# hzeller/timg

Hardware: NVIDIA H100
Metric: Mpixels/s scale+dither+sixel-encode @4K→cell (higher is better)
Workload: dtype u8/f32

## Files before the change

timg_b200/csrc/sixel.cu:

```cuda
#include <cstdlib>

#include "sixel.cuh"

namespace b200timg {

constexpr int PT = 1024;

__device__ __forceinline__ int pick_plane(int d0, int d1, int d2) {
    const double lum[3] = {0.2989, 0.5866, 0.1145};
    const int spreads[3] = {d0 << 3, d1 << 3, d2 << 3};
    int plane = 0; double best = 0.0;
#pragma unroll
    for (int p = 0; p < 3; ++p) { const double sp = lum[p] * (double)spreads[p]; if (sp > best) { plane = p; best = sp; } }
    return plane;
}

template <bool SMEM_TABLES>
__global__ void __launch_bounds__(PT)
sixel_palette_kernel(const uint32_t *__restrict__ fb, int w, int h, SixelWork W) {
    extern __shared__ uint32_t s_hist[];
    __shared__ uint32_t s_w[PT / 32];
    __shared__ int b_ind[256], b_col[256], b_med[256], t_ind[256], t_col[256], t_med[256];
    __shared__ uint32_t b_sum[256], b_low[256], t_sum[256], t_low[256];
    __shared__ int s_mn[3], s_mx[3];
// ... 349 lines not shown
constexpr int DW_MAX = 24;
constexpr int DCH = 16;
constexpr int DIN_STRIDE = DCH + 1;
constexpr int DOUT_STRIDE = 20;
constexpr int DWARP_SMEM = 2 * 32 * DIN_STRIDE * 4 + 32 * DOUT_STRIDE;

__global__ void __launch_bounds__(DW_MAX * 32)
sixel_dither_kernel(const uint32_t *__restrict__ fb, int w, int h, int nwarps, SixelWork W) {
    extern __shared__ __align__(16) uint8_t s_dyn[];
    __shared__ uint32_t s_pal[256];
    __shared__ volatile int s_progress[2048];
    const int f = blockIdx.x;
    const SixelFrameHdr *hdr = W.hdr + f;
    if (!hdr->diffuse) return;
    const int tid = threadIdx.x, lane = tid & 31, wid = tid >> 5;
    const int nthreads = nwarps * 32;
    uint8_t *s_lut = s_dyn;
    for (int i = tid; i < 32768 / 4; i += nthreads)
        reinterpret_cast<uint32_t *>(s_lut)[i] = reinterpret_cast<const uint32_t *>(W.lut + (long long)f * 32768)[i];
    for (int i = tid; i < 256; i += nthreads) s_pal[i] = hdr->palette[i];
    for (int i = tid; i < W.nb32; i += nthreads) s_progress[i] = 0;
    __syncthreads();
    uint32_t *s_in = reinterpret_cast<uint32_t *>(s_dyn + 32768 + (size_t)wid * DWARP_SMEM);
    uint8_t *s_out = reinterpret_cast<uint8_t *>(s_in + 2 * 32 * DIN_STRIDE);
    const uint32_t *frame = fb + (long long)f * w * h;
    uint8_t *index = W.index + (long long)f * w * h;
    uint32_t *bnd = W.boundary + (long long)f * W.nb32 * w;
    const int hrow = lane >> 4, hcol = lane & 15;

    for (int band = wid; band < W.nb32; band += nwarps) {
        const int y = band * 32 + lane;
        const bool row_ok = y < h;
        const bool last_row = (y == h - 1);
        const uint32_t *bin = band > 0 ? bnd + (long long)(band - 1) * w : nullptr;
        uint32_t *bout = bnd + (long long)band * w;
        uint32_t last_e = EZ;
        FsErr up_m1, up_0, up_p1, own, e_first;
        up_m1.zero(); up_0.zero(); up_p1.zero(); own.zero(); e_first.zero();
        const int steps = w + 62, nchunks = (steps + DCH - 1) / DCH;
        uint32_t pre[16];
        auto load_chunk = [&](int c) {
#pragma unroll
            for (int i = 0; i < 16; ++i) {
                const int r = 2 * i + hrow, yy = band * 32 + r, x = c * DCH - 2 * r + hcol;
                pre[i] = (yy < h && x >= 0 && x < w) ? frame[(long long)yy * w + x] : 0u;
            }
        };
        auto store_chunk = [&](int c) {
            uint32_t *t = s_in + (c & 1) * 32 * DIN_STRIDE;
#pragma unroll
            for (int i = 0; i < 16; ++i) t[(2 * i + hrow) * DIN_STRIDE + hcol] = pre[i];
        };
        load_chunk(0); store_chunk(0);
        __syncwarp();
        for (int c = 0; c < nchunks; ++c) {
            const int t0 = c * DCH;
            if (c + 1 < nchunks) load_chunk(c + 1);
            uint32_t binreg = EZ;
            if (band > 0) {
                const int need = min(w, t0 + DCH + 1);
                if (lane == 0) { while (s_progress[band - 1] < need) __nanosleep(32); __threadfence_block(); }
                __syncwarp();
                const int bx = t0 + 1 + lane;
                if (lane < DCH && bx < w) binreg = __ldcg(bin + bx);
                if (c == 0 && lane == 0) up_p1.unpack(__ldcg(bin));
            }
            const uint32_t *tin = s_in + (c & 1) * 32 * DIN_STRIDE + lane * DIN_STRIDE;
            uint32_t bkeep = EZ;
            const bool interior = (t0 - 62 >= 1) && (t0 + DCH - 1 <= w - 2) && (band * 32 + 31 < h - 1);
            if (interior) {
#pragma unroll 4
                for (int j = 0; j < DCH; ++j) {
                    uint32_t recv = __shfl_up_sync(0xffffffffu, last_e, 1);
                    const uint32_t b0 = __shfl_sync(0xffffffffu, binreg, j);
                    if (lane == 0) recv = b0;
                    up_m1 = up_0; up_0 = up_p1; up_p1.unpack(recv);
                    const uint32_t px = tin[j];
                    int v[3] = {(int)(px & 0xff), (int)((px >> 8) & 0xff), (int)((px >> 16) & 0xff)};
#pragma unroll
                    for (int ch = 0; ch < 3; ++ch) {
                        v[ch] = fs_add(v[ch], up_m1, ch, 1);
                        v[ch] = fs_add(v[ch], up_0, ch, 5);
                        v[ch] = fs_add(v[ch], up_p1, ch, 3);
                        v[ch] = fs_add(v[ch], own, ch, 7);
                    }
                    const uint32_t cell = ((uint32_t)(v[0] >> 3) << 10) | ((uint32_t)(v[1] >> 3) << 5) | (uint32_t)(v[2] >> 3);
                    const uint32_t ci = s_lut[cell];
                    const uint32_t pal = s_pal[ci];
                    own.set(v[0] - (int)(pal & 0xff), v[1] - (int)((pal >> 8) & 0xff), v[2] - (int)((pal >> 16) & 0xff));
                    last_e = own.pack();
                    s_out[lane * DOUT_STRIDE + j] = (uint8_t)ci;
                    const uint32_t e31 = __shfl_sync(0xffffffffu, last_e, 31);
                    if (lane == j) bkeep = e31;
                }
            } else {
#pragma unroll 2
                for (int j = 0; j < DCH; ++j) {
                    const int t = t0 + j, x = t - 2 * lane;
                    uint32_t recv = __shfl_up_sync(0xffffffffu, last_e, 1);
                    const uint32_t b0 = __shfl_sync(0xffffffffu, binreg, j);
                    if (lane == 0) recv = b0;
                    up_m1 = up_0; up_0 = up_p1; up_p1.unpack(recv);
                    uint32_t ci = 0;
                    if (x >= 0 && x < w && row_ok) {
                        const uint32_t px = tin[j];
                        int v[3] = {(int)(px & 0xff), (int)((px >> 8) & 0xff), (int)((px >> 16) & 0xff)};
#pragma unroll
                        for (int ch = 0; ch < 3; ++ch) {
                            v[ch] = fs_add(v[ch], up_m1, ch, 1);
                            v[ch] = fs_add(v[ch], up_0, ch, 5);
                            v[ch] = fs_add(v[ch], up_p1, ch, 3);
                            if (x == w - 1) v[ch] = fs_add(v[ch], e_first, ch, 3);
                            v[ch] = fs_add(v[ch], own, ch, 7);
                        }
                        const uint32_t cell = ((uint32_t)(v[0] >> 3) << 10) | ((uint32_t)(v[1] >> 3) << 5) | (uint32_t)(v[2] >> 3);
                        ci = s_lut[cell];
                        const uint32_t pal = s_pal[ci];
                        if (x < w - 1 && !last_row) own.set(v[0] - (int)(pal & 0xff), v[1] - (int)((pal >> 8) & 0xff), v[2] - (int)((pal >> 16) & 0xff));
                        else own.zero();
                        if (x == 0) e_first = own;
                        last_e = own.pack();
                    } else if (x >= w) {
                        last_e = EZ;
                    }
                    s_out[lane * DOUT_STRIDE + j] = (uint8_t)ci;
                    const uint32_t e31 = __shfl_sync(0xffffffffu, last_e, 31);
                    if (lane == j) bkeep = e31;
                }
            }
            __syncwarp();
#pragma unroll
            for (int i = 0; i < 16; ++i) {
                const int r = 2 * i + hrow, yy = band * 32 + r, x = t0 - 2 * r + hcol;
                if (yy < h && x >= 0 && x < w) index[(long long)yy * w + x] = s_out[r * DOUT_STRIDE + hcol];
            }
            {
                const int x = t0 + lane - 62;
                if (lane < DCH && x >= 0 && x < w) __stcg(bout + x, bkeep);
                __threadfence_block();
                __syncwarp();
                const int done = min(w, t0 + DCH - 62);
                if (lane == 0 && done > 0) s_progress[band] = done;
            }
            if (c + 1 < nchunks) store_chunk(c + 1);
            __syncwarp();
        }
    }
}

__device__ __forceinline__ uint32_t ndig4(uint32_t v) { return 1u + (v >= 10u) + (v >= 100u) + (v >= 1000u); }
__device__ __forceinline__ char *put_num4(char *o, uint32_t v) {
    const uint32_t d3 = v / 1000u, r3 = v - d3 * 1000u, d2 = r3 / 100u, r2 = r3 - d2 * 100u, d1 = r2 / 10u, d0 = r2 - d1 * 10u;
    if (v >= 1000u) *o++ = (char)('0' + d3);
    if (v >= 100u) *o++ = (char)('0' + d2);
    if (v >= 10u) *o++ = (char)('0' + d1);
    *o++ = (char)('0' + d0);
    return o;
}
__device__ __forceinline__ uint32_t rle_len(uint32_t n) { return n > 3u ? 2u + ndig4(n) : n; }
__device__ __forceinline__ char *put_rle(char *o, uint32_t n, char ch) {
    if (n > 3u) { *o++ = '!'; o = put_num4(o, n); *o++ = ch; }
    else { if (n > 0u) *o++ = ch; if (n > 1u) *o++ = ch; if (n > 2u) *o++ = ch; }
    return o;
}

constexpr int ET = 512, EW = ET / 32;
__device__ __forceinline__ uint32_t ent_pack(uint32_t c, uint32_t x, uint32_t bits) { return (c << 18) | (x << 6) | bits; }

struct EmitGeom { int w, h, cols_per_warp; };

template <typename F>
__device__ __forceinline__ void walk_runs(const uint32_t *sorted, int lo, int hi, int n, F emit) {
    int i = lo;
    uint32_t prev = 0; bool have_prev = false;
    if (i > 0 && i < hi) { prev = sorted[i - 1]; have_prev = true; }
    while (i < hi) {
        const uint32_t e = sorted[i];
        if (have_prev && e == prev + 64u) { prev = e; ++i; continue; }
        uint32_t cur = e, L = 1;
        while (i + (int)L < n && sorted[i + L] == cur + 64u) { cur += 64u; ++L; }
        const uint32_t c = e >> 18, x = (e >> 6) & 4095u;
        const bool same_colour = have_prev && (prev >> 18) == c;
        emit(c, e & 63u, same_colour ? x - ((prev >> 6) & 4095u) - 1u : x, L, !same_colour);
        prev = cur; have_prev = true;
        i += (int)L;
    }
}

__global__ void __launch_bounds__(ET)
sixel_emit_kernel(EmitGeom G, SixelWork W) {
    extern __shared__ uint32_t s_sorted[];
    __shared__ uint32_t s_cnt[EW][256];
    __shared__ uint32_t s_mask[EW * 256];
    __shared__ uint32_t s_w[ET / 32];
    const int band = blockIdx.x, f = blockIdx.y, tid = threadIdx.x, lane = tid & 31, wid = tid >> 5;
    const int w = G.w;
    const SixelFrameHdr *hdr = W.hdr + f;
    const uint8_t *idx = W.index + ((long long)f * G.h + (long long)band * 6) * w;

    for (int i = tid; i < EW * 256; i += ET) { (&s_cnt[0][0])[i] = 0; s_mask[i] = 0; }
    __syncthreads();

    const int x_lo = wid * G.cols_per_warp, x_hi = min(w, x_lo + G.cols_per_warp);
    uint32_t *cnt = s_cnt[wid];
    for (int x = x_lo + lane; x < x_hi; x += 32) {
        uint32_t col[6], bits[6];
        const uint32_t valid = column_entries(idx, w, x, col, bits);
#pragma unroll
        for (int s = 0; s < 6; ++s) if (valid & (1u << s)) atomicAdd(&cnt[col[s]], 1u);
    }
    __syncthreads();
    uint32_t tot_c = 0;
    if (tid < 256) for (int k = 0; k < EW; ++k) tot_c += s_cnt[k][tid];
    uint32_t n_ent; const uint32_t cb = block_excl_scan<ET>(tid < 256 ? tot_c : 0, s_w, n_ent);
    if (tid < 256) {
        uint32_t run = cb;
        for (int k = 0; k < EW; ++k) { const uint32_t v = s_cnt[k][tid]; s_cnt[k][tid] = run; run += v; }
    }
    __syncthreads();
    uint32_t *M = s_mask + wid * 256;
    const uint32_t lt = (1u << lane) - 1;
    for (int x0 = x_lo; x0 < x_hi; x0 += 32) {
        const int x = x0 + lane;
        uint32_t col[6], bits[6];
        const uint32_t valid = x < x_hi ? column_entries(idx, w, x, col, bits) : 0u;
#pragma unroll
        for (int s = 0; s < 6; ++s) if (valid & (1u << s)) atomicOr(&M[col[s]], 1u << lane);
        __syncwarp();
        uint32_t mk[6];
#pragma unroll
        for (int s = 0; s < 6; ++s)
            if (valid & (1u << s)) {
                mk[s] = M[col[s]];
                s_sorted[cnt[col[s]] + __popc(mk[s] & lt)] = ent_pack(col[s], (uint32_t)x, bits[s]);
            }
        __syncwarp();
#pragma unroll
        for (int s = 0; s < 6; ++s)
            if ((valid & (1u << s)) && (mk[s] & lt) == 0) { cnt[col[s]] += (uint32_t)__popc(mk[s]); M[col[s]] = 0; }
        __syncwarp();
    }
    __syncthreads();
    const int n = (int)n_ent;
    const uint32_t minc = s_sorted[0] >> 18;
    const int per = (n + ET - 1) / ET, lo = min(n, tid * per), hi = min(n, lo + per);
    uint32_t local = 0;
    walk_runs(s_sorted, lo, hi, n, [&](uint32_t c, uint32_t, uint32_t gap, uint32_t len, bool first) {
        local += rle_len(gap) + rle_len(len) + (first ? 1u + ndig4(c) + (c != minc ? 1u : 0u) : 0u);
    });
    uint32_t band_total; uint32_t at = block_excl_scan<ET>(local, s_w, band_total);
    if (tid == 0) W.band_bytes[(long long)f * W.nbands + band] = band_total;
    char *o = W.scratch + ((size_t)f * W.nbands + band) * W.band_cap + at;
    walk_runs(s_sorted, lo, hi, n, [&](uint32_t c, uint32_t bits, uint32_t gap, uint32_t len, bool first) {
        if (first) { if (c != minc) *o++ = '$'; *o++ = '#'; o = put_num4(o, c); }
        o = put_rle(o, gap, '?');
        o = put_rle(o, len, (char)('?' + bits));
    });
}

constexpr int SLOT_WORDS = 22;
constexpr int STASH_STEPS = 6;
constexpr uint32_t SLOT_MAX = 4 * (SLOT_WORDS - 3);
static_assert(SLOT_WORDS * ET >= 2 * EW * 256, "the slots alias the sort's tables");

struct DecTable { uint32_t v[4096]; };
constexpr DecTable make_dec_table() {
    DecTable t{};
    for (uint32_t n = 0; n < 4096; ++n) {
        uint32_t s = 0, m = n, nd = 0;
        do { s = (s << 8) | (0x30u + m % 10u); m /= 10u; ++nd; } while (m);
        t.v[n] = s;
    }
    return t;
}
__device__ const DecTable k_dec = make_dec_table();
__device__ __forceinline__ uint32_t dec4(uint32_t v, uint32_t &nd) {
    const uint32_t s = __ldg(&k_dec.v[v]);
    nd = 4u - ((uint32_t)__clz((int)s) >> 3);
    return s;
}
__device__ __forceinline__ unsigned long long rle_piece4(uint32_t n, uint32_t ch, uint32_t &len) {
    if (n > 3u) {
        uint32_t nd;
        const uint32_t d = dec4(n, nd);
        len = 2u + nd;
        return 0x21ull | ((unsigned long long)d << 8) | ((unsigned long long)ch << (8u * (1u + nd)));
    }
    len = n;
    return (unsigned long long)((ch * 0x010101u) & ((1u << (8u * n)) - 1u));
}
__device__ __forceinline__ void slot_append(uint32_t *slot, uint32_t &pos, uint32_t &cur, unsigned long long v, uint32_t len) {
    const uint32_t sh = 8u * (pos & 3u);
    const uint32_t lo = (uint32_t)v, hi = (uint32_t)(v >> 32);
    const uint32_t w0 = cur | (lo << sh);
    const uint32_t w1 = __funnelshift_l(lo, hi, sh);
    const uint32_t w2 = sh ? (hi >> (32u - sh)) : 0u;
    uint32_t *p = slot + min(pos >> 2, (uint32_t)(SLOT_WORDS - 3)) * ET;
    p[0] = w0; p[ET] = w1; p[2 * ET] = w2;
    const uint32_t np = pos + len, adv = (np >> 2) - (pos >> 2);
    cur = adv == 0u ? w0 : (adv == 1u ? w1 : w2);
    pos = np;
}

__global__ void __launch_bounds__(ET, 2)
sixel_emit1b_kernel(EmitGeom G, SixelWork W) {
    extern __shared__ uint32_t s_sorted[];
    __shared__ uint32_t s_tab[SLOT_WORDS * ET];
    __shared__ uint32_t s_w[ET / 32];
    const int band = blockIdx.x, f = blockIdx.y, tid = threadIdx.x, lane = tid & 31, wid = tid >> 5;
    const int w = G.w;
    const uint8_t *idx = W.index + ((long long)f * G.h + (long long)band * 6) * w;

    for (int i = tid; i < 2 * EW * 256; i += ET) s_tab[i] = 0;
    __syncthreads();
    const int x_lo = wid * G.cols_per_warp, x_hi = min(w, x_lo + G.cols_per_warp);
    uint32_t *cnt = s_tab + wid * 256, *M = s_tab + EW * 256 + wid * 256;
    const bool stash = G.cols_per_warp <= 32 * STASH_STEPS;
    uint32_t k0[STASH_STEPS], k1[STASH_STEPS], k2[STASH_STEPS];
    if (stash) {
#pragma unroll
        for (int t = 0; t < STASH_STEPS; ++t) {
            const int x = x_lo + 32 * t + lane;
            k0[t] = k1[t] = k2[t] = 0;
            if (x < x_hi) {
                uint32_t col[6], bits[6];
                const uint32_t valid = column_entries(idx, w, x, col, bits);
#pragma unroll
                for (int s = 0; s < 6; ++s) if (valid & (1u << s)) atomicAdd(&cnt[col[s]], 1u);
                k0[t] = col[0] | (col[1] << 8) | (col[2] << 16) | (col[3] << 24);
                k1[t] = col[4] | (col[5] << 8) | (valid << 16) | (bits[5] << 22);
                k2[t] = bits[0] | (bits[1] << 6) | (bits[2] << 12) | (bits[3] << 18) | (bits[4] << 24);
            }
        }
    } else {
        for (int x = x_lo + lane; x < x_hi; x += 32) {
            uint32_t col[6], bits[6];
            const uint32_t valid = column_entries(idx, w, x, col, bits);
#pragma unroll
            for (int s = 0; s < 6; ++s) if (valid & (1u << s)) atomicAdd(&cnt[col[s]], 1u);
        }
    }
    __syncthreads();
    uint32_t tot_c = 0;
    if (tid < 256) for (int k = 0; k < EW; ++k) tot_c += s_tab[k * 256 + tid];
    uint32_t n_ent; const uint32_t cb = block_excl_scan<ET>(tid < 256 ? tot_c : 0, s_w, n_ent);
    if (tid < 256) {
        uint32_t run = cb;
        for (int k = 0; k < EW; ++k) { const uint32_t v = s_tab[k * 256 + tid]; s_tab[k * 256 + tid] = run; run += v; }
    }
    __syncthreads();
    const uint32_t lt = (1u << lane) - 1;
    auto scatter_step = [&](int x, uint32_t valid, const uint32_t *col, const uint32_t *bits) {
#pragma unroll
        for (int s = 0; s < 6; ++s) if (valid & (1u << s)) atomicOr(&M[col[s]], 1u << lane);
        __syncwarp();
        uint32_t mk[6];
#pragma unroll
        for (int s = 0; s < 6; ++s)
            if (valid & (1u << s)) {
                mk[s] = M[col[s]];
                s_sorted[cnt[col[s]] + __popc(mk[s] & lt)] = ent_pack(col[s], (uint32_t)x, bits[s]);
            }
        __syncwarp();
#pragma unroll
        for (int s = 0; s < 6; ++s)
            if ((valid & (1u << s)) && (mk[s] & lt) == 0) { cnt[col[s]] += (uint32_t)__popc(mk[s]); M[col[s]] = 0; }
        __syncwarp();
    };
    if (stash) {
#pragma unroll
        for (int t = 0; t < STASH_STEPS; ++t) {
            if (x_lo + 32 * t < x_hi) {
                const uint32_t col[6] = {k0[t] & 255u, (k0[t] >> 8) & 255u, (k0[t] >> 16) & 255u, k0[t] >> 24, k1[t] & 255u, (k1[t] >> 8) & 255u};
                const uint32_t bits[6] = {k2[t] & 63u, (k2[t] >> 6) & 63u, (k2[t] >> 12) & 63u, (k2[t] >> 18) & 63u, (k2[t] >> 24) & 63u, (k1[t] >> 22) & 63u};
                scatter_step(x_lo + 32 * t + lane, (k1[t] >> 16) & 63u, col, bits);
            }
        }
    } else {
        for (int x0 = x_lo; x0 < x_hi; x0 += 32) {
            const int x = x0 + lane;
            uint32_t col[6], bits[6];
            const uint32_t valid = x < x_hi ? column_entries(idx, w, x, col, bits) : 0u;
            scatter_step(x, valid, col, bits);
        }
    }
    __syncthreads();
    const int n = (int)n_ent;
    const uint32_t minc = s_sorted[0] >> 18;
    const int per = (n + ET - 1) / ET, lo = min(n, tid * per), hi = min(n, lo + per);
    uint32_t *slot = s_tab + tid;
    uint32_t pos = 0, cur = 0;
    bool ovf = false;
    walk_runs(s_sorted, lo, hi, n, [&](uint32_t c, uint32_t bits, uint32_t gap, uint32_t len, bool first) {
        uint32_t pl;
        if (first) {
            uint32_t nd;
            unsigned long long v = 0x23ull | ((unsigned long long)dec4(c, nd) << 8);
            pl = 1u + nd;
            if (c != minc) { v = 0x24ull | (v << 8); ++pl; }
            ovf |= pos > SLOT_MAX;
            slot_append(slot, pos, cur, v, pl);
        }
        uint32_t rl;
        const unsigned long long gv = rle_piece4(gap, 0x3fu, pl), rv = rle_piece4(len, 0x3fu + bits, rl);
        ovf |= pos > SLOT_MAX;
        if (pl + rl <= 8u) {
            slot_append(slot, pos, cur, gv | (rv << (8u * pl)), pl + rl);
        } else {
            slot_append(slot, pos, cur, gv, pl);
            ovf |= pos > SLOT_MAX;
            slot_append(slot, pos, cur, rv, rl);
        }
    });
    const uint32_t local = pos;
    uint32_t band_total; const uint32_t at = block_excl_scan<ET>(local, s_w, band_total);
    if (tid == 0) W.band_bytes[(long long)f * W.nbands + band] = band_total;
    char *o = W.scratch + ((size_t)f * W.nbands + band) * W.band_cap + at;
    if (!ovf) {
        const uint32_t head = min(local, (4u - (at & 3u)) & 3u);
        const uint32_t w0 = slot[0];
        for (uint32_t k = 0; k < head; ++k) o[k] = (char)(w0 >> (8u * k));
        const uint32_t nw = (local - head) >> 2;
        uint32_t *dw = reinterpret_cast<uint32_t *>(o + head);
        uint32_t a = w0;
        for (uint32_t j = 0; j < nw; ++j) {
            const uint32_t b = slot[(j + 1) * ET];
            dw[j] = __funnelshift_r(a, b, 8u * head);
            a = b;
        }
        const uint32_t done = head + 4u * nw;
        for (uint32_t k = done; k < local; ++k) o[k] = (char)(slot[(k >> 2) * ET] >> (8u * (k & 3u)));
    } else {
        walk_runs(s_sorted, lo, hi, n, [&](uint32_t c, uint32_t bits, uint32_t gap, uint32_t len, bool first) {
            if (first) { if (c != minc) *o++ = '$'; *o++ = '#'; o = put_num4(o, c); }
            o = put_rle(o, gap, '?');
            o = put_rle(o, len, (char)('?' + bits));
        });
    }
}

__global__ void __launch_bounds__(256)
sixel_layout_kernel(int w, int h, SixelWork W) {
    __shared__ uint32_t s_w[8];
    __shared__ uint32_t s_carry;
    const int f = blockIdx.x, tid = threadIdx.x;
    SixelFrameHdr *hdr = W.hdr + f;
    uint32_t len = 0;
    if ((uint32_t)tid < hdr->ncolors) {
        const uint32_t p = hdr->palette[tid];
        const uint32_t r = ((p & 0xff) * 100 + 127) / 255, g = (((p >> 8) & 0xff) * 100 + 127) / 255, b = (((p >> 16) & 0xff) * 100 + 127) / 255;
        len = 1 + ndig_u((uint32_t)tid) + 3 + ndig_u(r) + 1 + ndig_u(g) + 1 + ndig_u(b);
    }
    uint32_t pal_total; (void)block_excl_scan<256>(len, s_w, pal_total);
    const uint32_t header = 8 + ndig_u((uint32_t)w) + 1 + ndig_u((uint32_t)h) + pal_total;
    if (tid == 0) s_carry = header;
    __syncthreads();
    uint32_t *bb = W.band_bytes + (long long)f * W.nbands;
    for (int b0 = 0; b0 < W.nbands; b0 += 256) {
        const int b = b0 + tid;
        const uint32_t v = b < W.nbands ? bb[b] + (b > 0 ? 1u : 0u) : 0;
        uint32_t tot; const uint32_t at = block_excl_scan<256>(v, s_w, tot);
        if (b < W.nbands) W.band_off[(long long)f * W.nbands + b] = s_carry + at + (b > 0 ? 1u : 0u);
        __syncthreads();
        if (tid == 0) s_carry += tot;
        __syncthreads();
    }
    if (tid == 0) { hdr->header_len = header; hdr->frame_size = s_carry + 2; }
}

__global__ void __launch_bounds__(1024)
sixel_sizes_to_offsets_kernel(const SixelFrameHdr *__restrict__ hdr, int n, uint64_t *__restrict__ offsets) {
    __shared__ unsigned long long s_wv[32];
    __shared__ unsigned long long c_run;
    const int tid = threadIdx.x, lane = tid & 31, wid = tid >> 5;
    if (tid == 0) c_run = 0;
    __syncthreads();
    for (int i0 = 0; i0 < n; i0 += 1024) {
        const int i = i0 + tid;
        unsigned long long v = i < n ? hdr[i].frame_size : 0ull;
        const unsigned long long mine = v;
#pragma unroll
        for (int d = 1; d < 32; d <<= 1) { const unsigned long long o = __shfl_up_sync(0xffffffffu, v, d); if (lane >= d) v += o; }
        if (lane == 31) s_wv[wid] = v;
        __syncthreads();
        unsigned long long pre = 0, tot = 0;
        for (int k = 0; k < 32; ++k) { if (k < wid) pre += s_wv[k]; tot += s_wv[k]; }
        if (i < n) offsets[i] = c_run + pre + v - mine;
        __syncthreads();
        if (tid == 0) c_run += tot;
        __syncthreads();
    }
    if (tid == 0) offsets[n] = c_run;
}

__global__ void __launch_bounds__(256)
sixel_compact_kernel(int w, int h, SixelWork W, const uint64_t *__restrict__ offsets, char *__restrict__ out,
                     unsigned long long out_cap) {
    __shared__ uint32_t s_w[8];
    const int band = blockIdx.x, f = blockIdx.y, tid = threadIdx.x;
    const SixelFrameHdr *hdr = W.hdr + f;
    const unsigned long long fbase = offsets[f];
    if (fbase + hdr->frame_size > out_cap) return;
    const uint32_t boff = W.band_off[(long long)f * W.nbands + band];
    const uint32_t n = W.band_bytes[(long long)f * W.nbands + band];
    const char *src = W.scratch + ((size_t)f * W.nbands + band) * W.band_cap;
    char *dst = out + fbase + boff;
    {
        const uint32_t head = min(n, (uint32_t)((4 - (reinterpret_cast<uintptr_t>(dst) & 3)) & 3));
        if ((uint32_t)tid < head) dst[tid] = src[tid];
        const uint32_t nw = (n - head) >> 2, m = head & 3;
        const uint32_t *sw = reinterpret_cast<const uint32_t *>(src + head - m);
        uint32_t *dw = reinterpret_cast<uint32_t *>(dst + head);
        for (uint32_t j = tid; j < nw; j += 256) dw[j] = m ? __funnelshift_r(sw[j], sw[j + 1], 8 * m) : sw[j];
        const uint32_t done = head + (nw << 2);
        if (done + tid < n) dst[done + tid] = src[done + tid];
    }
    if (tid == 0) {
        if (band > 0) dst[-1] = '-';
        if (band == W.nbands - 1) { out[fbase + hdr->frame_size - 2] = '\033'; out[fbase + hdr->frame_size - 1] = '\\'; }
    }
    if (band == 0) {
        if (tid == 0) {
            char *o = out + fbase;
            *o++ = '\033'; *o++ = 'P'; *o++ = 'q'; *o++ = '"'; *o++ = '1'; *o++ = ';'; *o++ = '1'; *o++ = ';';
            o = put_num_u(o, (uint32_t)w); *o++ = ';'; o = put_num_u(o, (uint32_t)h);
        }
        const uint32_t fixed = 8 + ndig_u((uint32_t)w) + 1 + ndig_u((uint32_t)h);
        uint32_t len = 0, r = 0, g = 0, b = 0;
        if ((uint32_t)tid < hdr->ncolors) {
            const uint32_t p = hdr->palette[tid];
            r = ((p & 0xff) * 100 + 127) / 255; g = (((p >> 8) & 0xff) * 100 + 127) / 255; b = (((p >> 16) & 0xff) * 100 + 127) / 255;
            len = 1 + ndig_u((uint32_t)tid) + 3 + ndig_u(r) + 1 + ndig_u(g) + 1 + ndig_u(b);
        }
        uint32_t tot; const uint32_t at = block_excl_scan<256>(len, s_w, tot);
        if (len) {
            char *q = out + fbase + fixed + at;
            *q++ = '#'; q = put_num_u(q, (uint32_t)tid); *q++ = ';'; *q++ = '2'; *q++ = ';';
            q = put_num_u(q, r); *q++ = ';'; q = put_num_u(q, g); *q++ = ';'; q = put_num_u(q, b);
        }
    }
}

static size_t align_up(size_t v, size_t a) { return (v + a - 1) / a * a; }

struct SixelPlan {
    SixelWork W;
    bool emit_v1, dither_v1;
    int emit_mode;
    EmitGeom G;
    size_t emit_smem, o_d2_bnd, o_d2_prog;
    long long npix;
};

static int sixel_plan(b200timg_ctx *ctx, int w, int h, int n_frames, bool reserve, SixelPlan *S) {
    if (h % 6) return ctx->fail(B200TIMG_EINVAL, "sixel: height %d is not a multiple of 6", h);
    if (n_frames > 65535) return ctx->fail(B200TIMG_EINVAL, "sixel: too many frames for one launch");
    SixelWork &W = S->W;
    const long long npix = (long long)w * h;
    S->npix = npix;
    long long step_px = npix / 18383; if (npix < 18383) step_px = 6; if (step_px == 0) step_px = 1;
    const long long ns = (npix + step_px - 1) / step_px;
    W.ent_cap = (int)std::min<long long>(32768, ns);
    W.nb32 = (h + 31) / 32; W.nbands = h / 6;
    if (W.nb32 > 2048) return ctx->fail(B200TIMG_EINVAL, "sixel: frame too tall");
    size_t off = 0;
    const size_t o_hdr = off; off += align_up(sizeof(SixelFrameHdr) * n_frames, 256);
    const size_t o_ea = off; off += align_up(sizeof(uint32_t) * (size_t)W.ent_cap * n_frames, 256);
    const size_t o_eb = off; off += align_up(sizeof(uint32_t) * (size_t)W.ent_cap * n_frames, 256);
    const size_t o_lut = off; off += align_up((size_t)32768 * n_frames, 256);
    const size_t o_idx = off; off += align_up((size_t)npix * n_frames, 256);
    const size_t o_bnd = off; off += align_up(sizeof(uint32_t) * (size_t)W.nb32 * w * n_frames, 256);
    const size_t o_bb = off; off += align_up(sizeof(uint32_t) * (size_t)W.nbands * n_frames, 256);
    const size_t o_bo = off; off += align_up(sizeof(uint32_t) * (size_t)W.nbands * n_frames, 256);
    W.band_cap = align_up((size_t)w * 42 + 256 * 5 + 16, 256);
    const size_t o_scr = off;
    {
        const bool v1_fits = w <= 4095 && sizeof(uint32_t) * (size_t)6 * w <= (size_t)(227 - 36) * 1024;
        const bool v1b_fits = w <= 4095 && sizeof(uint32_t) * (size_t)6 * w <= (size_t)(227 - 47) * 1024;
        int mode = v1b_fits ? 4 : v1_fits ? 1 : 2;
        if (getenv("B200TIMG_EMIT_V2")) mode = 2;
        if (const char *e = getenv("B200TIMG_EMIT")) mode = atoi(e);
        if (mode < 1 || mode > 4 || (mode == 1 && !v1_fits) || (mode == 4 && !v1b_fits)) mode = 2;
        S->emit_mode = mode;
        S->emit_v1 = mode == 1 || mode == 4;
    }
    if (S->emit_v1) off += W.band_cap * W.nbands * n_frames;
    S->dither_v1 = getenv("B200TIMG_DITHER_V1") != nullptr;
    size_t d_bnd, d_prog;
    const size_t o_d2 = off; off += sixel_dither_workspace(w, h, n_frames, &d_bnd, &d_prog);
    size_t e_hdr, e_desc, e_ctl;
    const size_t o_e2 = off; off += sixel_emit_workspace(w, h, n_frames, &e_hdr, &e_desc, &e_ctl);
    if (reserve) B2_CUDA(ctx, ctx->sixel_work.reserve(off));
    if (!ctx->sixel_work.p || ctx->sixel_work.cap < off) return ctx->fail(B200TIMG_EINVAL, "sixel: write phase without prepare");
    ctx->sixel_idx_off = o_idx;
    char *base = ctx->sixel_work.as<char>();
    W.hdr = reinterpret_cast<SixelFrameHdr *>(base + o_hdr);
    W.ent_a = reinterpret_cast<uint32_t *>(base + o_ea); W.ent_b = reinterpret_cast<uint32_t *>(base + o_eb);
    W.lut = reinterpret_cast<uint8_t *>(base + o_lut); W.index = reinterpret_cast<uint8_t *>(base + o_idx);
    W.boundary = reinterpret_cast<uint32_t *>(base + o_bnd); W.band_bytes = reinterpret_cast<uint32_t *>(base + o_bb);
    W.band_off = reinterpret_cast<uint32_t *>(base + o_bo); W.scratch = base + o_scr;
    W.hdr_bytes = base + o_e2 + e_hdr;
    W.desc = reinterpret_cast<unsigned long long *>(base + o_e2 + e_desc);
    W.ctl = reinterpret_cast<uint32_t *>(base + o_e2 + e_ctl);
    S->o_d2_bnd = o_d2 + d_bnd; S->o_d2_prog = o_d2 + d_prog;
    S->G.w = w; S->G.h = h; S->G.cols_per_warp = ((w + EW - 1) / EW + 31) / 32 * 32;
    const size_t smem_limit = 227 * 1024 - 36 * 1024;
    S->emit_smem = sizeof(uint32_t) * (size_t)6 * w;
    if (!ctx->sixel_attrs_set) {
        B2_CUDA(ctx, cudaFuncSetAttribute(sixel_palette_kernel<false>, cudaFuncAttributeMaxDynamicSharedMemorySize, 65536));
        B2_CUDA(ctx, cudaFuncSetAttribute(sixel_emit_kernel, cudaFuncAttributeMaxDynamicSharedMemorySize, (int)smem_limit));
        B2_CUDA(ctx, cudaFuncSetAttribute(sixel_emit1b_kernel, cudaFuncAttributeMaxDynamicSharedMemorySize, (227 - 47) * 1024));
        B2_CUDA(ctx, cudaFuncSetAttribute(sixel_dither_kernel, cudaFuncAttributeMaxDynamicSharedMemorySize, 32768 + DW_MAX * DWARP_SMEM));
        B2_CUDA(ctx, cudaFuncSetAttribute(sixel_palette_kernel<true>, cudaFuncAttributeMaxDynamicSharedMemorySize, 200 * 1024));
        ctx->sixel_attrs_set = true;
    }
    return B200TIMG_OK;
}

int launch_sixel_front(b200timg_ctx *ctx, const uint8_t *d_fb, int w, int h, int n_total, int f0, int n, bool reserve) {
    if ((reinterpret_cast<uintptr_t>(d_fb) & 3)) return ctx->fail(B200TIMG_EINVAL, "sixel: framebuffer must be 4-byte aligned");
    SixelPlan S;
    B2_TRY(sixel_plan(ctx, w, h, n_total, reserve, &S));
    SixelWork W = S.W;
    const long long npix = S.npix;
    W.hdr += f0; W.ent_a += (long long)f0 * W.ent_cap; W.ent_b += (long long)f0 * W.ent_cap; W.lut += (long long)f0 * 32768;
    W.index += (long long)f0 * npix; W.boundary += (long long)f0 * W.nb32 * w;
    W.band_bytes += (long long)f0 * W.nbands; W.band_off += (long long)f0 * W.nbands;
    W.scratch += (size_t)f0 * W.nbands * W.band_cap;
    const uint32_t *fb = reinterpret_cast<const uint32_t *>(d_fb) + (long long)f0 * npix;
    char *base = ctx->sixel_work.as<char>();
    B2_KERNEL(ctx, "sixel_palette_kernel");
    {
        const size_t t_words = W.ent_cap > 16384 ? (size_t)W.ent_cap : 16384;
        const size_t smem_tables = sizeof(uint32_t) * (t_words + (size_t)W.ent_cap);
        if (smem_tables <= 200 * 1024) sixel_palette_kernel<true><<<n, PT, smem_tables, ctx->stream>>>(fb, w, h, W);
        else sixel_palette_kernel<false><<<n, PT, 65536, ctx->stream>>>(fb, w, h, W);
    }
    B2_LAUNCH_CHECK(ctx);
    B2_KERNEL(ctx, "sixel_lut_kernel");
    sixel_lut_kernel<<<dim3(128, n), 256, 0, ctx->stream>>>(W);
    B2_LAUNCH_CHECK(ctx);
    {
        long long blocks = (npix + 255) / 256; if (blocks > 64) blocks = 64;
        B2_KERNEL(ctx, "sixel_map_kernel");
        sixel_map_kernel<<<dim3((unsigned)blocks, n), 256, 0, ctx->stream>>>(fb, npix, W);
        B2_LAUNCH_CHECK(ctx);
    }
    if (!S.dither_v1) {
        B2_TRY(launch_sixel_dither(ctx, fb, w, h, n, n_total, W, base + S.o_d2_bnd + sizeof(uint4) * (size_t)f0 * W.nb32 * w,
                                   base + S.o_d2_prog + sizeof(int) * (size_t)f0 * W.nb32));
    } else {
        B2_KERNEL(ctx, "sixel_dither_kernel");
        const int rounds = (W.nb32 + DW_MAX - 1) / DW_MAX;
        const int nwarps = (W.nb32 + rounds - 1) / rounds;
        const size_t dsmem = 32768 + (size_t)nwarps * DWARP_SMEM;
        sixel_dither_kernel<<<n, nwarps * 32, dsmem, ctx->stream>>>(fb, w, h, nwarps, W);
        B2_LAUNCH_CHECK(ctx);
    }
    if (S.emit_v1) {
        B2_KERNEL(ctx, "sixel_emit_kernel");
        if (S.emit_mode == 4) sixel_emit1b_kernel<<<dim3(W.nbands, n), ET, S.emit_smem, ctx->stream>>>(S.G, W);
        else sixel_emit_kernel<<<dim3(W.nbands, n), ET, S.emit_smem, ctx->stream>>>(S.G, W);
        B2_LAUNCH_CHECK(ctx);
    }
    return B200TIMG_OK;
}

int launch_sixel_back(b200timg_ctx *ctx, int w, int h, int n_frames, char *d_out, size_t out_cap, uint64_t *d_offsets, int phases) {
    SixelPlan S;
    B2_TRY(sixel_plan(ctx, w, h, n_frames, false, &S));
    const SixelWork &W = S.W;
    if (!S.emit_v1) {
        if (!(phases & 2)) return B200TIMG_OK;
        if (S.emit_mode == 2) return launch_sixel_emit(ctx, w, h, n_frames, W, d_out, out_cap, d_offsets);
        return launch_sixel_emit3(ctx, w, h, n_frames, W, d_out, out_cap, d_offsets);
    }
    if (phases & 1) {
        B2_KERNEL(ctx, "sixel_layout_kernel");
        sixel_layout_kernel<<<n_frames, 256, 0, ctx->stream>>>(w, h, W);
        B2_LAUNCH_CHECK(ctx);
        B2_KERNEL(ctx, "sixel_sizes_to_offsets_kernel");
        sixel_sizes_to_offsets_kernel<<<1, 1024, 0, ctx->stream>>>(W.hdr, n_frames, d_offsets);
        B2_LAUNCH_CHECK(ctx);
    }
    if (!(phases & 2)) return B200TIMG_OK;
    B2_KERNEL(ctx, "sixel_compact_kernel");
    sixel_compact_kernel<<<dim3(W.nbands, n_frames), 256, 0, ctx->stream>>>(w, h, W, d_offsets, d_out, (unsigned long long)out_cap);
    B2_LAUNCH_CHECK(ctx);
    return B200TIMG_OK;
}

int launch_sixel(b200timg_ctx *ctx, const uint8_t *d_fb, int w, int h, int n_frames, char *d_out,
                 size_t out_cap, uint64_t *d_offsets, int phases) {
    if (phases & 1) B2_TRY(launch_sixel_front(ctx, d_fb, w, h, n_frames, 0, n_frames, true));
    return launch_sixel_back(ctx, w, h, n_frames, d_out, out_cap, d_offsets, phases);
}

int sixel_debug_fetch(b200timg_ctx *ctx, uint32_t *h_palette, uint32_t *h_counts, uint8_t *h_index, size_t index_bytes) {
    if (!ctx->sixel_work.p) return ctx->fail(B200TIMG_EINVAL, "sixel: nothing encoded yet");
    SixelFrameHdr host;
    B2_CUDA(ctx, cudaMemcpyAsync(&host, ctx->sixel_work.p, sizeof host, cudaMemcpyDeviceToHost, ctx->stream));
    if (h_index && index_bytes)
        B2_CUDA(ctx, cudaMemcpyAsync(h_index, ctx->sixel_work.as<char>() + ctx->sixel_idx_off, index_bytes,
                                     cudaMemcpyDeviceToHost, ctx->stream));
    B2_CUDA(ctx, cudaStreamSynchronize(ctx->stream));
    if (h_palette) memcpy(h_palette, host.palette, sizeof host.palette);
    if (h_counts) { h_counts[0] = host.ncolors; h_counts[1] = host.origcolors; }
    return B200TIMG_OK;
}

}
```

Measured before the change: 69810.

## Stage band index rows in shared memory and coalesce band output via smem image

Adds a V5 variant of the 1b emit kernel, made the default mode. It loads the six index rows of a band into shared memory with coalesced word reads before the histogram pass, replacing scattered byte reads from global memory. At the end it assembles the encoded band in shared memory and copies it to global memory with 16-byte stores instead of per-thread unaligned word writes. It also adds optional clock64 phase instrumentation behind a compile flag. The risks are extra synchronisation and more register pressure from the per-thread row buffer.

Result: faster. 71910 (median of 6 runs) (+3.0%).

```diff
diff --git a/timg_b200/csrc/sixel.cu b/timg_b200/csrc/sixel.cu
--- a/timg_b200/csrc/sixel.cu
+++ b/timg_b200/csrc/sixel.cu
@@ -675,6 +675,22 @@
     pos = np;
 }
 
+#ifdef B200TIMG_EMIT_CLOCKS
+constexpr int EMIT_CLK_PHASES = 8;
+__device__ unsigned long long g_emit_clocks[2][EMIT_CLK_PHASES];
+#define EMIT_CLK_BEGIN long long clk_[EMIT_CLK_PHASES + 1]; int clk_n_ = 0; if (threadIdx.x == 0) clk_[clk_n_] = clock64(); ++clk_n_
+#define EMIT_CLK() do { __syncthreads(); if (threadIdx.x == 0) clk_[clk_n_] = clock64(); ++clk_n_; } while (0)
+#define EMIT_CLK_END(kern) do { if (threadIdx.x == 0) for (int k_ = 0; k_ + 1 < clk_n_; ++k_) \
+        atomicAdd(&g_emit_clocks[kern][k_], (unsigned long long)(clk_[k_ + 1] - clk_[k_])); } while (0)
+#else
+#define EMIT_CLK_BEGIN do {} while (0)
+#define EMIT_CLK() do {} while (0)
+#define EMIT_CLK_END(kern) do {} while (0)
+#endif
+
+constexpr int ROW_WORDS = (6 * 32 * STASH_STEPS * EW + 3) / 4 / ET + 1;
+
+template <bool V5>
 __global__ void __launch_bounds__(ET, 2)
 sixel_emit1b_kernel(EmitGeom G, SixelWork W) {
     extern __shared__ uint32_t s_sorted[];
@@ -683,12 +699,27 @@
     const int band = blockIdx.x, f = blockIdx.y, tid = threadIdx.x, lane = tid & 31, wid = tid >> 5;
     const int w = G.w;
     const uint8_t *idx = W.index + ((long long)f * G.h + (long long)band * 6) * w;
-
-    for (int i = tid; i < 2 * EW * 256; i += ET) s_tab[i] = 0;
-    __syncthreads();
+    EMIT_CLK_BEGIN;
+    const bool stash = G.cols_per_warp <= 32 * STASH_STEPS;
+    const uint8_t *cols = idx;
+    if (V5 && stash) {
+        const uint32_t a = (uint32_t)(reinterpret_cast<uintptr_t>(idx) & 3u);
+        const uint32_t *gw = reinterpret_cast<const uint32_t *>(idx - a);
+        const int nw = (int)((a + 6u * (uint32_t)w + 3u) >> 2);
+        uint32_t rw[ROW_WORDS];
+#pragma unroll
+        for (int k = 0; k < ROW_WORDS; ++k) { const int j = tid + k * ET; rw[k] = j < nw ? gw[j] : 0u; }
+        for (int i = tid; i < 2 * EW * 256; i += ET) s_tab[i] = 0;
+#pragma unroll
+        for (int k = 0; k < ROW_WORDS; ++k) { const int j = tid + k * ET; if (j < nw) s_sorted[j] = rw[k]; }
+        cols = reinterpret_cast<const uint8_t *>(s_sorted) + a;
+    } else {
+        for (int i = tid; i < 2 * EW * 256; i += ET) s_tab[i] = 0;
+    }
+    __syncthreads();
+    if (!V5) EMIT_CLK();
     const int x_lo = wid * G.cols_per_warp, x_hi = min(w, x_lo + G.cols_per_warp);
     uint32_t *cnt = s_tab + wid * 256, *M = s_tab + EW * 256 + wid * 256;
-    const bool stash = G.cols_per_warp <= 32 * STASH_STEPS;
     uint32_t k0[STASH_STEPS], k1[STASH_STEPS], k2[STASH_STEPS];
     if (stash) {
 #pragma unroll
@@ -697,7 +728,7 @@
             k0[t] = k1[t] = k2[t] = 0;
             if (x < x_hi) {
                 uint32_t col[6], bits[6];
-                const uint32_t valid = column_entries(idx, w, x, col, bits);
+                const uint32_t valid = column_entries(cols, w, x, col, bits);
 #pragma unroll
                 for (int s = 0; s < 6; ++s) if (valid & (1u << s)) atomicAdd(&cnt[col[s]], 1u);
                 k0[t] = col[0] | (col[1] << 8) | (col[2] << 16) | (col[3] << 24);
@@ -714,6 +745,7 @@
         }
     }
     __syncthreads();
+    EMIT_CLK();
     uint32_t tot_c = 0;
     if (tid < 256) for (int k = 0; k < EW; ++k) tot_c += s_tab[k * 256 + tid];
     uint32_t n_ent; const uint32_t cb = block_excl_scan<ET>(tid < 256 ? tot_c : 0, s_w, n_ent);
@@ -722,6 +754,7 @@
         for (int k = 0; k < EW; ++k) { const uint32_t v = s_tab[k * 256 + tid]; s_tab[k * 256 + tid] = run; run += v; }
     }
     __syncthreads();
+    EMIT_CLK();
     const uint32_t lt = (1u << lane) - 1;
     auto scatter_step = [&](int x, uint32_t valid, const uint32_t *col, const uint32_t *bits) {
 #pragma unroll
@@ -758,6 +791,7 @@
         }
     }
     __syncthreads();
+    EMIT_CLK();
     const int n = (int)n_ent;
     const uint32_t minc = s_sorted[0] >> 18;
     const int per = (n + ET - 1) / ET, lo = min(n, tid * per), hi = min(n, lo + per);
@@ -786,15 +820,18 @@
         }
     });
     const uint32_t local = pos;
+    EMIT_CLK();
     uint32_t band_total; const uint32_t at = block_excl_scan<ET>(local, s_w, band_total);
     if (tid == 0) W.band_bytes[(long long)f * W.nbands + band] = band_total;
-    char *o = W.scratch + ((size_t)f * W.nbands + band) * W.band_cap + at;
-    if (!ovf) {
+    EMIT_CLK();
+    char *const band_out = W.scratch + ((size_t)f * W.nbands + band) * W.band_cap;
+    char *o = band_out + at;
+    auto slot_out = [&](char *d) {
         const uint32_t head = min(local, (4u - (at & 3u)) & 3u);
         const uint32_t w0 = slot[0];
-        for (uint32_t k = 0; k < head; ++k) o[k] = (char)(w0 >> (8u * k));
+        for (uint32_t k = 0; k < head; ++k) d[k] = (char)(w0 >> (8u * k));
         const uint32_t nw = (local - head) >> 2;
-        uint32_t *dw = reinterpret_cast<uint32_t *>(o + head);
+        uint32_t *dw = reinterpret_cast<uint32_t *>(d + head);
         uint32_t a = w0;
         for (uint32_t j = 0; j < nw; ++j) {
             const uint32_t b = slot[(j + 1) * ET];
@@ -802,7 +839,20 @@
             a = b;
         }
         const uint32_t done = head + 4u * nw;
-        for (uint32_t k = done; k < local; ++k) o[k] = (char)(slot[(k >> 2) * ET] >> (8u * (k & 3u)));
+        for (uint32_t k = done; k < local; ++k) d[k] = (char)(slot[(k >> 2) * ET] >> (8u * (k & 3u)));
+    };
+    if (V5 && !__syncthreads_or(ovf) && band_total <= 24u * (uint32_t)w) {
+        char *img = reinterpret_cast<char *>(s_sorted);
+        slot_out(img + at);
+        __syncthreads();
+        const uint32_t n16 = band_total >> 4;
+        const uint4 *s16 = reinterpret_cast<const uint4 *>(img);
+        uint4 *d16 = reinterpret_cast<uint4 *>(band_out);
+        for (uint32_t j = tid; j < n16; j += ET) d16[j] = s16[j];
+        const uint32_t t = (n16 << 4) + (uint32_t)tid;
+        if (t < band_total) band_out[t] = img[t];
+    } else if (!ovf) {
+        slot_out(o);
     } else {
         walk_runs(s_sorted, lo, hi, n, [&](uint32_t c, uint32_t bits, uint32_t gap, uint32_t len, bool first) {
             if (first) { if (c != minc) *o++ = '$'; *o++ = '#'; o = put_num4(o, c); }
@@ -810,6 +860,8 @@
             o = put_rle(o, len, (char)('?' + bits));
         });
     }
+    EMIT_CLK();
+    EMIT_CLK_END(V5 ? 1 : 0);
 }
 
 __global__ void __launch_bounds__(256)
@@ -950,12 +1002,12 @@
     {
         const bool v1_fits = w <= 4095 && sizeof(uint32_t) * (size_t)6 * w <= (size_t)(227 - 36) * 1024;
         const bool v1b_fits = w <= 4095 && sizeof(uint32_t) * (size_t)6 * w <= (size_t)(227 - 47) * 1024;
-        int mode = v1b_fits ? 4 : v1_fits ? 1 : 2;
+        int mode = v1b_fits ? 5 : v1_fits ? 1 : 2;
         if (getenv("B200TIMG_EMIT_V2")) mode = 2;
         if (const char *e = getenv("B200TIMG_EMIT")) mode = atoi(e);
-        if (mode < 1 || mode > 4 || (mode == 1 && !v1_fits) || (mode == 4 && !v1b_fits)) mode = 2;
+        if (mode < 1 || mode > 5 || (mode == 1 && !v1_fits) || (mode >= 4 && !v1b_fits)) mode = 2;
         S->emit_mode = mode;
-        S->emit_v1 = mode == 1 || mode == 4;
+        S->emit_v1 = mode == 1 || mode >= 4;
     }
     if (S->emit_v1) off += W.band_cap * W.nbands * n_frames;
     S->dither_v1 = getenv("B200TIMG_DITHER_V1") != nullptr;
@@ -982,7 +1034,8 @@
     if (!ctx->sixel_attrs_set) {
         B2_CUDA(ctx, cudaFuncSetAttribute(sixel_palette_kernel<false>, cudaFuncAttributeMaxDynamicSharedMemorySize, 65536));
         B2_CUDA(ctx, cudaFuncSetAttribute(sixel_emit_kernel, cudaFuncAttributeMaxDynamicSharedMemorySize, (int)smem_limit));
-        B2_CUDA(ctx, cudaFuncSetAttribute(sixel_emit1b_kernel, cudaFuncAttributeMaxDynamicSharedMemorySize, (227 - 47) * 1024));
+        B2_CUDA(ctx, cudaFuncSetAttribute(sixel_emit1b_kernel<false>, cudaFuncAttributeMaxDynamicSharedMemorySize, (227 - 47) * 1024));
+        B2_CUDA(ctx, cudaFuncSetAttribute(sixel_emit1b_kernel<true>, cudaFuncAttributeMaxDynamicSharedMemorySize, (227 - 47) * 1024));
         B2_CUDA(ctx, cudaFuncSetAttribute(sixel_dither_kernel, cudaFuncAttributeMaxDynamicSharedMemorySize, 32768 + DW_MAX * DWARP_SMEM));
         B2_CUDA(ctx, cudaFuncSetAttribute(sixel_palette_kernel<true>, cudaFuncAttributeMaxDynamicSharedMemorySize, 200 * 1024));
         ctx->sixel_attrs_set = true;
@@ -1031,8 +1084,9 @@
         B2_LAUNCH_CHECK(ctx);
     }
     if (S.emit_v1) {
-        B2_KERNEL(ctx, "sixel_emit_kernel");
-        if (S.emit_mode == 4) sixel_emit1b_kernel<<<dim3(W.nbands, n), ET, S.emit_smem, ctx->stream>>>(S.G, W);
+        B2_KERNEL(ctx, S.emit_mode == 5 ? "sixel_emit5_kernel" : "sixel_emit_kernel");
+        if (S.emit_mode == 5) sixel_emit1b_kernel<true><<<dim3(W.nbands, n), ET, S.emit_smem, ctx->stream>>>(S.G, W);
+        else if (S.emit_mode == 4) sixel_emit1b_kernel<false><<<dim3(W.nbands, n), ET, S.emit_smem, ctx->stream>>>(S.G, W);
         else sixel_emit_kernel<<<dim3(W.nbands, n), ET, S.emit_smem, ctx->stream>>>(S.G, W);
         B2_LAUNCH_CHECK(ctx);
     }
@@ -1083,3 +1137,14 @@
 }
 
 }
+
+#ifdef B200TIMG_EMIT_CLOCKS
+extern "C" int b200timg_emit_clocks(unsigned long long *out) {
+    using b200timg::g_emit_clocks;
+    static const unsigned long long zero[2][b200timg::EMIT_CLK_PHASES] = {};
+    if (cudaDeviceSynchronize() != cudaSuccess || cudaMemcpyFromSymbol(out, g_emit_clocks, sizeof zero) != cudaSuccess ||
+        cudaMemcpyToSymbol(g_emit_clocks, zero, sizeof zero) != cudaSuccess)
+        return -3;
+    return 0;
+}
+#endif
```
